# ztlpn/minilp

Hardware: AMD Instinct MI355X
Metric: simplex pivots/sec (higher is better)
Workload: dtype f64; 1 GPU; config 4: random LP 100000 vars x 100000 constraints, 100 nnz/row (0.1% fill), Max c'x, Ax<=b, x>=0; primal simplex with PSE+DSE from the slack basis; timed pivots 5..1983; parallelism=1 GPU, nucleus_size_at_end=1559, completed_steps=1978

## Files before the change

### minilp_amd/csrc/kernels.hip

```cpp
#include "kernels.h"
#include <hip/hip_ext.h>

#include <limits.h>
#include <math.h>

#include <cstdlib>
#include <string>

namespace mlp {

#define NONE_IDX INT_MAX
constexpr int BLK = 256;

struct Cand {
    double key;
    int idx;
};
__device__ __forceinline__ Cand cand_none() { return Cand{-INFINITY, NONE_IDX}; }
__device__ __forceinline__ bool cand_better(const Cand& a, const Cand& b) {
    return a.key > b.key || (a.key == b.key && a.idx < b.idx);
}
__device__ __forceinline__ Cand wave_best(Cand c) {
#pragma unroll
    for (int o = 32; o > 0; o >>= 1) {
// ... 711 lines not shown
            v.tau[r] = inv * inv;
        }
        int base = v.csr_ptr[i_r], end = v.csr_ptr[i_r + 1];
        int cnt = 0;
        for (int e0 = base; e0 < end; e0 += 128) {
            int sx[2] = {-1, -1}, cx[2], lx[2];
            double ax[2];
            bool vx[2];
#pragma unroll
            for (int h = 0; h < 2; ++h) {
                const int e = e0 + 64 * h + lane;
                vx[h] = e < end;
                cx[h] = vx[h] ? v.csr_col[e] : 0;
                ax[h] = vx[h] ? v.csr_val[e] : 0.0;
            }
#pragma unroll
            for (int h = 0; h < 2; ++h) lx[h] = v.var_loc[cx[h]];
#pragma unroll
            for (int h = 0; h < 2; ++h) {
                const int ks = v.kslot_of_pos[lx[h] >= 0 ? lx[h] : 0];
                if (vx[h] && lx[h] >= 0) sx[h] = ks;
            }
#pragma unroll
            for (int h = 0; h < 2; ++h) {
                if (h == 1 && e0 + 64 >= end) break;
                const int s = sx[h];
                bool isk = vx[h] && s >= 0;
                unsigned long long mask = __ballot(isk);
                const double coef = -ax[h] * inv;
                if (isk) {
                    int off = cnt + __popcll(mask & ((1ull << lane) - 1ull));
                    v.blist_s[off] = s;
                    v.blist_a[off] = coef;
                    if (l_n && off < RK_LDS) {
                        l_s[off] = s;
                        l_a[off] = coef;
                    }
                }
                cnt += __popcll(mask);
                if (nlow > 0) lr_dot_listed(mask, s, coef, Urow, lane < nlow, lr_acc);
            }
        }
        if (lane == 0) {
            it->blist_n = cnt;
            if (l_n) *l_n = cnt;
        }
    }
    if (nlow > 0) {
        if (sr >= 0 && lane < nlow) lr_acc = Urow[sr];
        if (lane < nlow) c->lr_e[lane] = lr_acc;
    }
    if (plan_after && lane == 0) plan_update(v, c, phase);
}

__device__ __forceinline__ Cand price_primal_one(double dd, double gm, uint8_t f, int j, int use_pse) {
    if (((f & NB_AT_MIN) && dd > -EPS) || ((f & NB_AT_MAX) && dd < EPS)) return cand_none();
    return Cand{use_pse ? dd * dd / gm : fabs(dd), j};
}
__device__ __forceinline__ Cand price_dual_one(double val, double mn, double mx, double bt, int r, int use_dse) {
    double infeas;
    if (val < mn - EPS) infeas = mn - val;
    else if (val > mx + EPS) infeas = val - mx;
    else return cand_none();
    return Cand{use_dse ? infeas * infeas / bt : infeas, r};
}
__device__ __forceinline__ void open_iteration(Ctl* c, int phase, Cand best) {
    IterState* it = &c->it;
    it->klist_n = 0;
    it->blist_n = 0;
    c->up.kase = -1;
    if (best.idx == NONE_IDX) {
        it->status = phase == 0 ? ITER_OPTIMAL : ITER_FEASIBLE;
        it->q = -1;
        it->r = -1;
        c->halt = 1;
        push_rec(c, phase);
    } else {
        it->status = ITER_PIVOT;
        if (phase == 0) {
            it->q = best.idx;
            it->r = -1;
        } else {
            it->r = best.idx;
            it->q = -1;
        }
    }
}
__device__ __forceinline__ void close_and_open(const DevView& v, Ctl* c, int phase, Cand best, double pay, bool close_current) {
    __shared__ double s_key, s_pay;
    __shared__ int s_idx, s_go;
    if (threadIdx.x == 0) {
        if (close_current) push_rec(c, phase);
        if (close_current && v.str_on) {
            c->hyper_epoch += 1;
            c->str_n = 0;
            c->aq_n = 0;
        }
        s_go = 1;
        if (close_current && c->forced) {
            c->halt = 1;
            s_go = 0;
        }
        s_key = best.key;
        s_idx = best.idx;
        s_pay = pay;
    }
    __syncthreads();
    if (!s_go || threadIdx.x >= 64) return;
    Cand b{s_key, s_idx};
    bool ok = true;
    if (phase == 0) ok = exchange_best_wave(v, c, phase, b, s_pay, threadIdx.x);
    else if (threadIdx.x == 0) ok = adopt_rank0_candidate(v, c, b);
    if (threadIdx.x == 0 && ok) open_iteration(c, phase, b);
}
__global__ void __launch_bounds__(BLK) k_price_primal(DevView v, int use_pse) {
    Ctl* c = v.ctl;
    if (c->halt) return;
    Cand best = cand_none();
    double pay = 0.0;
    for (int j = v.nb_lo + blockIdx.x * BLK + threadIdx.x; j < v.nb_hi; j += gridDim.x * BLK) {
        double dj = v.d[j];
        Cand t = price_primal_one(dj, use_pse ? v.gamma[j] : 1.0, v.nbflags[j], j, use_pse);
        if (cand_better(t, best)) {
            best = t;
            pay = dj;
        }
    }
    if (!grid_best_p(best, pay, v)) return;
    close_and_open(v, c, 0, best, pay, false);
}
__global__ void __launch_bounds__(BLK) k_price_dual(DevView v, int use_dse) {
    Ctl* c = v.ctl;
    if (c->halt || c->forced) return;
    Cand best = cand_none();
    for (int r = blockIdx.x * BLK + threadIdx.x; r < v.m; r += gridDim.x * BLK) {
        Cand t = price_dual_one(v.xB[r], v.loB[r], v.hiB[r], use_dse ? v.beta[r] : 1.0, r, use_dse);
        if (cand_better(t, best)) best = t;
    }
    if (!grid_best(best, v)) return;
    if (threadIdx.x == 0 && adopt_rank0_candidate(v, c, best)) open_iteration(c, 1, best);
}

__global__ void __launch_bounds__(64) k_ftran_prep(DevView v, int derive_primal) {
    Ctl* c = v.ctl;
    if (c->halt || c->it.status != ITER_PIVOT) {
        if (threadIdx.x == 0) c->side_go = 0;
        return;
    }
    if (threadIdx.x == 0) c->side_go = 1;
    KMARK0(c, 0);
    ftran_prep_wave(v, c, threadIdx.x, derive_primal);
}
template <int G>
__device__ __forceinline__ void push_F(const DevView& v, int p, double x, double* out_pos, int gl, Ctl* list_ctl = nullptr) {
    int var = v.basic_vars[p];
    int end = v.csc_ptr[var + 1];
    for (int e = v.csc_ptr[var] + gl; e < end; e += G) {
        const RowInfo ri = v.rowinfo[v.csc_row[e]];
        if (ri.kslot < 0) {
            unsafeAtomicAdd(&out_pos[ri.pos], -v.csc_val[e] * x / ri.diag);
            if (list_ctl) aq_list_add(v, list_ctl, ri.pos);
        }
    }
}
template <int G>
__device__ __forceinline__ void mark_F(const DevView& v, int p, int gl) {
    const int var = v.basic_vars[p];
    const int end = v.csc_ptr[var + 1];
    for (int e = v.csc_ptr[var] + gl; e < end; e += G) {
        const RowInfo ri = v.rowinfo[v.csc_row[e]];
        if (ri.kslot < 0) v.fmark[ri.pos] = 1;
    }
}
template <int G>
__global__ void __launch_bounds__(BLK) k_ftran_gather(DevView v) {
    Ctl* c = v.ctl;
    if (c->halt || c->it.status != ITER_PIVOT) return;
    KMARK0(c, 18);
    int slot = (blockIdx.x * BLK + threadIdx.x) / G;
    int gl = threadIdx.x & (G - 1);
    if (slot >= c->k) return;
    int n = c->it.klist_n;
    double acc = 0.0;
    const double* wrow = v.W + (size_t)slot * v.ld;
    if (G == 4) {
        for (int j0 = gl; j0 < n; j0 += 16) {
            double a[4], w[4];
            int si[4];
#pragma unroll
            for (int u = 0; u < 4; ++u) {
                const int j = j0 + 4 * u;
                a[u] = j < n ? v.klist_a[j] : 0.0;
                si[u] = j < n ? v.klist_s[j] : 0;
            }
#pragma unroll
            for (int u = 0; u < 4; ++u) w[u] = j0 + 4 * u < n ? wrow[si[u]] : 0.0;
#pragma unroll
            for (int u = 0; u < 4; ++u)
                if (j0 + 4 * u < n) acc += a[u] * w[u];
        }
        if (v.lrJ) {
            const int nlow = c->nlow;
            double e[LR_MAX / 4], x[LR_MAX / 4];
#pragma unroll
            for (int u = 0; u < LR_MAX / 4; ++u) {
                const int j = gl + 4 * u;
                e[u] = j < nlow ? c->lr_c[j] : 0.0;
                x[u] = j < nlow ? v.U[(size_t)j * v.ld + slot] : 0.0;
            }
#pragma unroll
            for (int u = 0; u < LR_MAX / 4; ++u)
                if (gl + 4 * u < nlow) acc += x[u] * e[u];
        }
    } else {
        for (int j = gl; j < n; j += G) acc += v.klist_a[j] * wrow[v.klist_s[j]];
        if (v.lrJ) {
            const int nlow = c->nlow;
            for (int j = gl; j < nlow; j += G) acc += v.U[(size_t)j * v.ld + slot] * c->lr_c[j];
        }
    }
    acc = group_sum<G>(acc);
    int p = v.pos_of_kslot[slot];
    if (gl == 0) {
        v.aK[slot] = acc;
        v.alpha_q[p] = acc;
        if (acc != 0.0 && aq_listing(v)) aq_list_add(v, c, p);
    }
    if (acc != 0.0 && !v.pb_on && !v.det_pull) push_F<G>(v, p, acc, v.alpha_q, gl, aq_listing(v) ? c : nullptr);
    else if (acc != 0.0 && v.det_pull && v.fmark) mark_F<G>(v, p, gl);
}

constexpr int PB_TILE = 512;
__global__ void __launch_bounds__(BLK) k_push_stage1(DevView v, int which) {
    Ctl* c = v.ctl;
    if (c->halt || c->it.status != ITER_PIVOT) return;
    KMARK0(c, 19);
    __shared__ double acc[PB_ROWS];
    __shared__ double s_x[PB_TILE];
    __shared__ int s_beg[PB_TILE], s_len[PB_TILE];
    int b = blockIdx.x, cc = blockIdx.y;
    if ((gridDim.y & 7) == 0) {
        const int L = (int)blockIdx.x + (int)gridDim.x * (int)blockIdx.y, idx = L >> 3;
        cc = (L & 7) + 8 * (idx / (int)gridDim.x);
        b = idx % (int)gridDim.x;
    }
    const int tid = threadIdx.x;
    const int row0 = b * PB_ROWS;
    const int nrows = min(PB_ROWS, v.m - row0);
    for (int t = tid; t < nrows; t += BLK) acc[t] = 0.0;
    const int k = c->k;
    const int per = (k + (int)gridDim.y - 1) / (int)gridDim.y;
    const int s_lo = cc * per, s_hi = min(k, s_lo + per);
    const double* xK = which ? v.tauK : v.aK;
    const int lane = tid & 7, grp = tid >> 3;
    const int stride = v.pb_rb + 1;
    for (int tile0 = s_lo; tile0 < s_hi; tile0 += PB_TILE) {
        const int nt = min(PB_TILE, s_hi - tile0);
        __syncthreads();
        for (int t = tid; t < nt; t += BLK) {
            const int slot = tile0 + t;
            const double x = xK[slot];
            const int var = v.basic_vars[v.pos_of_kslot[slot]];
            const int beg = v.colblk[(size_t)var * stride + b], end = v.colblk[(size_t)var * stride + b + 1];
            s_x[t] = x;
            s_beg[t] = beg;
            s_len[t] = (x != 0.0) ? end - beg : 0;
        }
        __syncthreads();
        for (int base = grp * 4; base < nt; base += (BLK / 8) * 4) {
            int r[4];
            double a[4];
#pragma unroll
            for (int j = 0; j < 4; ++j) {
                const int t = base + j;
                const int len = t < nt ? s_len[t] : 0;
                r[j] = -1;
                a[j] = 0.0;
                if (lane < len) {
                    const int e = s_beg[t] + lane;
                    r[j] = v.csc_row[e] - row0;
                    a[j] = v.csc_val[e] * s_x[t];
                }
            }
#pragma unroll
            for (int j = 0; j < 4; ++j)
                if (r[j] >= 0) unsafeAtomicAdd(&acc[r[j]], a[j]);
#pragma unroll 1
            for (int j = 0; j < 4; ++j) {
                const int t = base + j;
                const int len = t < nt ? s_len[t] : 0;
                for (int o = 8 + lane; o < len; o += 8) {
                    const int e = s_beg[t] + o;
                    unsafeAtomicAdd(&acc[v.csc_row[e] - row0], v.csc_val[e] * s_x[t]);
                }
            }
        }
    }
    __syncthreads();
    double* dst = v.push_part + (size_t)cc * v.m + row0;
    for (int t = tid; t < nrows; t += BLK) dst[t] = acc[t];
}
constexpr int PBD_TILE = 256;
constexpr int PBD_CHUNKS_DEFAULT = 16;
constexpr size_t PBD_LDS = sizeof(unsigned long long) * 2 * PB_ROWS + sizeof(double) * PBD_TILE + sizeof(int) * 2 * PBD_TILE;
__global__ void __launch_bounds__(BLK) k_push_stage1_det(DevView v, int which) {
    Ctl* c = v.ctl;
    if (c->halt || c->it.status != ITER_PIVOT) return;
    KMARK0(c, 19);
    extern __shared__ unsigned long long s_pbd[];
    unsigned long long* accH = s_pbd;
    unsigned long long* accL = s_pbd + PB_ROWS;
    double* s_x = reinterpret_cast<double*>(s_pbd + 2 * PB_ROWS);
    int* s_beg = reinterpret_cast<int*>(s_x + PBD_TILE);
    int* s_len = s_beg + PBD_TILE;
    __shared__ double s_bound;
    int b = blockIdx.x, cc = blockIdx.y;
// ... 790 lines not shown
            c->it.max_step = max_step;
            c->it.alpha_sq = sq + 1.0;
            st_agent(&c->ratio_max_step, max_step);
            __hip_atomic_store(v.ticket, 0u, __ATOMIC_RELAXED, __HIP_MEMORY_SCOPE_AGENT);
            asm volatile("s_waitcnt vmcnt(0)" ::: "memory");
            st_agent(&c->ratio_epoch, epoch0 + 1);
        }
    }
    __shared__ int s_gave_up;
    if (threadIdx.x == 0) {
        s_gave_up = 0;
        long spins = 0;
        while (ld_agent(&c->ratio_epoch) != epoch0 + 1) {
            __builtin_amdgcn_s_sleep(1);
            if (++spins > c->ratio_spin_limit) {
                s_gave_up = 1;
                break;
            }
        }
        s_max_step = ld_agent(&c->ratio_max_step);
    }
    __syncthreads();
    if (s_gave_up) {
        if (threadIdx.x == 0 && atomicExch(&c->halt, 1) == 0) {
            c->it.status = ITER_STALL;
            push_rec(c, 0);
        }
        return;
    }
    const double max_step = s_max_step;
#pragma unroll
    for (int u = 0; u < PT; ++u) {
        if (pos[u] < 0) continue;
        if (stp[u] / ca[u] <= max_step) {
            Cand t{ca[u], pos[u]};
            if (cand_better(t, best)) best = t;
        }
    }
    if (!grid_best(best, v, nrb)) return;
    } while (0);
    ratio_primal_finish(v, c, best, rk_inside);
    KMARK(c, 6);
}

__global__ void __launch_bounds__(BLK) k_post_ftran(DevView v, int use_pse) {
    Ctl* c = v.ctl;
    if (c->halt || c->it.status != ITER_PIVOT) return;
    double sq = 0.0;
    if (use_pse) {
        for (int p = blockIdx.x * BLK + threadIdx.x; p < v.m; p += gridDim.x * BLK) {
            double coeff = v.alpha_q[p];
            sq += coeff * coeff;
            if (!v.fac_on && v.kslot_of_pos[p] < 0) v.rv[v.srow_of_pos[p]].y = coeff / v.sdiag_of_pos[p];
        }
    }
    if (!grid_sum(sq, v)) return;
    if (threadIdx.x == 0) {
        c->it.alpha_sq = sq + 1.0;
        plan_update(v, c, 1);
    }
}

__global__ void __launch_bounds__(64) k_btran_prep(DevView v, int derive_dual, int plan_after) {
    Ctl* c = v.ctl;
    if (c->halt || c->it.status != ITER_PIVOT) return;
    btran_prep_wave(v, c, threadIdx.x, c->it.r, derive_dual, plan_after, 1);
}
__device__ __forceinline__ void btran_rk_body(const DevView& v, Ctl* c, int block, int n_gather, int after_fold) {
    const int k = c->k;
    const int n = c->it.blist_n;
    double sq = 0.0;
    if (v.lrJ) {
        const int nlow = (after_fold && c->fold) ? 0 : c->nlow;
        for (int g4 = block * BLK + (int)threadIdx.x; g4 < 4 * k; g4 += n_gather * BLK) {
            const int s = g4 >> 2, gl = g4 & 3;
            double acc = 0.0;
            for (int j0 = gl; j0 < n; j0 += 16) {
                double a[4], w[4];
                int si[4];
#pragma unroll
                for (int u = 0; u < 4; ++u) {
                    const int j = j0 + 4 * u;
                    a[u] = j < n ? v.blist_a[j] : 0.0;
                    si[u] = j < n ? v.blist_s[j] : 0;
                }
#pragma unroll
                for (int u = 0; u < 4; ++u) w[u] = j0 + 4 * u < n ? v.W[(size_t)si[u] * v.ld + s] : 0.0;
#pragma unroll
                for (int u = 0; u < 4; ++u)
                    if (j0 + 4 * u < n) acc += a[u] * w[u];
            }
            {
                double e[LR_MAX / 4], x[LR_MAX / 4];
#pragma unroll
                for (int u = 0; u < LR_MAX / 4; ++u) {
                    const int j = gl + 4 * u;
                    e[u] = j < nlow ? c->lr_e[j] : 0.0;
                    x[u] = j < nlow ? v.V[(size_t)j * v.ld + s] : 0.0;
                }
#pragma unroll
                for (int u = 0; u < LR_MAX / 4; ++u)
                    if (gl + 4 * u < nlow) acc += e[u] * x[u];
            }
            acc += __shfl_xor(acc, 1, 64);
            acc += __shfl_xor(acc, 2, 64);
            if (gl == 0) {
                v.rK[s] = acc;
                v.rv[v.row_of_kslot[s]].x = acc;
                sq += acc * acc;
            }
        }
    } else
    for (int s = block * BLK + (int)threadIdx.x; s < k; s += n_gather * BLK) {
        double acc = 0.0;
        for (int j = 0; j < n; ++j) acc += v.blist_a[j] * v.W[(size_t)v.blist_s[j] * v.ld + s];
        v.rK[s] = acc;
        v.rv[v.row_of_kslot[s]].x = acc;
        sq += acc * acc;
    }
    if (!grid_sum(sq, v, n_gather, block)) return;
    if (threadIdx.x == 0) {
        int r = c->it.r;
        if (v.kslot_of_pos[r] < 0) {
            double inv = 1.0 / v.sdiag_of_pos[r];
            sq += inv * inv;
        }
        c->it.rho_sq = sq;
    }
}
template <int G>
__global__ void __launch_bounds__(BLK) k_btran(DevView v, int n_gather, int after_fold = 0) {
    Ctl* c = v.ctl;
    if (c->halt || c->it.status != ITER_PIVOT) return;
    KMARK0(c, 7);
    const int k = c->k;
    if ((int)blockIdx.x < n_gather) {
        btran_rk_body(v, c, (int)blockIdx.x, n_gather, after_fold);
    } else {
        int slot = (((int)blockIdx.x - n_gather) * BLK + threadIdx.x) / G;
        int gl = threadIdx.x & (G - 1);
        if (slot >= k) return;
        int p = v.pos_of_kslot[slot];
        int var = v.basic_vars[p];
        int end = v.csc_ptr[var + 1];
        double acc = 0.0;
        for (int e = v.csc_ptr[var] + gl; e < end; e += G) acc += v.csc_val[e] * v.rv[v.csc_row[e]].y;
        acc = group_sum<G>(acc);
        if (gl == 0) v.tK[slot] = v.alpha_q[p] - acc;
    }
}


constexpr int HEAD_CAP = 1024;
__device__ void ftran_head_lds(const DevView& v, Ctl* c, int lane, int derive_primal, bool primary, int* ls, double* la, int* ln) {
    IterState* it = &c->it;
    const int q = it->q;
    const int var = v.nb_vars[q];
    if (primary && lane == 0) {
        it->entering_var = var;
        if (derive_primal) {
            double dq = v.d[q];
            it->sign = dq < 0.0;
            it->entering_cur = v.xN[q];
            it->entering_other = (dq < 0.0) ? v.var_hi[var] : v.var_lo[var];
            it->r = -1;
            it->leaving_var = -1;
        }
    }
    const bool atomic_land = !v.pb_on && !v.det_pull;
    const int base = v.csc_ptr[var], end = v.csc_ptr[var + 1];
    int cnt = 0;
    for (int e0 = base; e0 < end; e0 += 64) {
        const int e = e0 + lane;
        const bool valid = e < end;
        int s = -1;
        double a = 0.0;
        if (valid) {
            const int i = v.csc_row[e];
            a = v.csc_val[e];
            s = v.kslot_of_row[i];
            if (s < 0 && primary) {
                const int p = v.pos_of_srow[i];
                const double x = a / v.sdiag_of_pos[p];
                if (atomic_land) unsafeAtomicAdd(&v.alpha_q[p], x);
                else v.alpha_q[p] = x;
                if (aq_listing(v)) aq_list_add(v, c, p);
            }
        }
        const bool isk = valid && s >= 0;
        const unsigned long long mask = __ballot(isk);
        if (isk) {
            const int off = cnt + __popcll(mask & ((1ull << lane) - 1ull));
            if (off < HEAD_CAP) {
                ls[off] = s;
                la[off] = a;
            }
            if (primary) {
                v.klist_s[off] = s;
                v.klist_a[off] = a;
            }
        }
        cnt += __popcll(mask);
    }
    if (lane == 0) {
        *ln = cnt < HEAD_CAP ? cnt : HEAD_CAP;
        if (primary) it->klist_n = cnt;
    }
}
__global__ void __launch_bounds__(BLK) k_ftran_gather_lrh(DevView v, int fpk) {
    Ctl* c = v.ctl;
    if (c->halt || c->it.status != ITER_PIVOT) {
        if (blockIdx.x == 0 && threadIdx.x == 0) c->side_go = 0;
        return;
    }
    KMARK0(c, 0);
    __shared__ int s_ls[HEAD_CAP];
    __shared__ double s_la[HEAD_CAP];
    __shared__ double s_lrc[LR_MAX];
    __shared__ int s_n;
    const bool primary = blockIdx.x == 0;
    const int nlow = c->nlow;
    if (threadIdx.x < 64) {
        const int lane = threadIdx.x;
        IterState* it = &c->it;
        const int q = it->q;
        const int var = v.nb_vars[q];
        if (primary && lane == 0) {
            c->side_go = 1;
            it->entering_var = var;
            const double dq = v.d[q];
            it->sign = dq < 0.0;
            it->entering_cur = v.xN[q];
            it->entering_other = (dq < 0.0) ? v.var_hi[var] : v.var_lo[var];
            it->r = -1;
            it->leaving_var = -1;
            c->fold = nlow >= v.lrJ ? 1 : 0;
        }
        const int base = v.csc_ptr[var], end = v.csc_ptr[var + 1];
        int cnt = 0;
        const double* Vrow = v.V + (size_t)(lane < nlow ? lane : 0) * v.ld;
        double lr_acc = 0.0;
        for (int e0 = base; e0 < end; e0 += 128) {
            int sx[2] = {-1, -1};
            double ax[2] = {0.0, 0.0};
            int ix[2];
            bool vx[2];
#pragma unroll
            for (int h = 0; h < 2; ++h) {
                const int e = e0 + 64 * h + lane;
                vx[h] = e < end;
                ix[h] = vx[h] ? v.csc_row[e] : 0;
                ax[h] = vx[h] ? v.csc_val[e] : 0.0;
            }
            RowInfo rx[2];
#pragma unroll
            for (int h = 0; h < 2; ++h) rx[h] = v.rowinfo[ix[h]];
#pragma unroll
            for (int h = 0; h < 2; ++h) {
                if (vx[h]) {
                    sx[h] = rx[h].kslot;
                    if (sx[h] < 0 && primary) v.alpha_q[rx[h].pos] = ax[h] / rx[h].diag;
                }
            }
#pragma unroll
            for (int h = 0; h < 2; ++h) {
                if (h == 1 && e0 + 64 >= end) break;
                const int s = sx[h];
                const double a = ax[h];
                const bool isk = vx[h] && s >= 0;
                const unsigned long long mask = __ballot(isk);
                if (isk) {
                    const int off = cnt + __popcll(mask & ((1ull << lane) - 1ull));
                    if (off < HEAD_CAP) {
                        s_ls[off] = s;
                        s_la[off] = a;
                    }
                    if (primary) {
                        v.klist_s[off] = s;
                        v.klist_a[off] = a;
                    }
                }
                cnt += __popcll(mask);
                if (nlow > 0) lr_dot_listed(mask, s, a, Vrow, lane < nlow, lr_acc);
            }
        }
        if (lane == 0) {
            s_n = cnt < HEAD_CAP ? cnt : HEAD_CAP;
            if (primary) it->klist_n = cnt;
        }
        if (lane < LR_MAX) s_lrc[lane] = lane < nlow ? lr_acc : 0.0;
        if (primary && lane < nlow) c->lr_c[lane] = lr_acc;
    }
    __syncthreads();
    const int slot = (blockIdx.x * BLK + threadIdx.x) / 4;
    const int gl = threadIdx.x & 3;
    if (slot >= c->k) return;
    const int n = s_n;
    double acc = 0.0;
    const double* wrow = v.W + (size_t)slot * v.ld;
    const int p = v.pos_of_kslot[slot];
    const int fvar = fpk ? v.basic_vars[p] : 0;
    for (int j0 = gl; j0 < n; j0 += 16) {
        double a[4], w[4];
        int si[4];
#pragma unroll
        for (int u = 0; u < 4; ++u) {
            const int j = j0 + 4 * u;
            a[u] = j < n ? s_la[j] : 0.0;
            si[u] = j < n ? s_ls[j] : 0;
        }
#pragma unroll
        for (int u = 0; u < 4; ++u) w[u] = j0 + 4 * u < n ? wrow[si[u]] : 0.0;
#pragma unroll
        for (int u = 0; u < 4; ++u)
            if (j0 + 4 * u < n) acc += a[u] * w[u];
    }
    {
        double e[LR_MAX / 4], x[LR_MAX / 4];
#pragma unroll
        for (int u = 0; u < LR_MAX / 4; ++u) {
            const int j = gl + 4 * u;
            e[u] = j < nlow ? s_lrc[j] : 0.0;
            x[u] = j < nlow ? v.U[(size_t)j * v.ld + slot] : 0.0;
        }
#pragma unroll
        for (int u = 0; u < LR_MAX / 4; ++u)
            if (gl + 4 * u < nlow) acc += x[u] * e[u];
    }
    acc = group_sum<4>(acc);
    if (gl == 0) {
        v.aK[slot] = acc;
        v.alpha_q[p] = acc;
        if (fpk) v.fpk_x[fvar] = acc;
    }
}
template <int G>
__global__ void __launch_bounds__(BLK) k_ftran_fused(DevView v, int derive_primal) {
    Ctl* c = v.ctl;
    if (c->halt || c->it.status != ITER_PIVOT) return;
    KMARK0(c, 0);
    __shared__ int s_ls[HEAD_CAP];
    __shared__ double s_la[HEAD_CAP];
    __shared__ int s_n;
    if (threadIdx.x < 64) ftran_head_lds(v, c, threadIdx.x, derive_primal, blockIdx.x == 0, s_ls, s_la, &s_n);
    __syncthreads();
    const int slot = (blockIdx.x * BLK + threadIdx.x) / G;
    const int gl = threadIdx.x & (G - 1);
    if (slot >= c->k) return;
    const int n = s_n;
    double acc = 0.0;
    const double* wrow = v.W + (size_t)slot * v.ld;
    for (int j = gl; j < n; j += G) acc += s_la[j] * wrow[s_ls[j]];
    acc = group_sum<G>(acc);
    const int p = v.pos_of_kslot[slot];
    if (gl == 0) {
        v.aK[slot] = acc;
        v.alpha_q[p] = acc;
        if (acc != 0.0 && aq_listing(v)) aq_list_add(v, c, p);
    }
    if (acc != 0.0 && !v.pb_on && !v.det_pull) push_F<G>(v, p, acc, v.alpha_q, gl, aq_listing(v) ? c : nullptr);
    else if (acc != 0.0 && v.det_pull && v.fmark) mark_F<G>(v, p, gl);
}
__device__ void btran_head_lds(const DevView& v, Ctl* c, int lane, int derive_dual, bool primary, int* ls, double* la, int* ln) {
    IterState* it = &c->it;
    const int r = it->r;
    if (derive_dual && !c->forced && primary && lane == 0) {
        const double val = v.xB[r], mn = v.loB[r];
        it->leaving_new_val = (val < mn) ? mn : v.hiB[r];
        it->leaving_var = v.basic_vars[r];
        it->q = -1;
        it->entering_var = -1;
    }
    const int sr = v.kslot_of_pos[r];
    if (sr >= 0) {
        if (lane == 0) {
            ls[0] = sr;
            la[0] = 1.0;
            *ln = 1;
            if (primary) {
                v.blist_s[0] = sr;
                v.blist_a[0] = 1.0;
                it->blist_n = 1;
            }
        }
        return;
    }
    const int i_r = v.srow_of_pos[r];
    const double inv = 1.0 / v.sdiag_of_pos[r];
    if (primary && lane == 0) {
        v.rv[i_r].x = inv;
        v.tau[r] = inv * inv;
    }
    const int base = v.csr_ptr[i_r], end = v.csr_ptr[i_r + 1];
    int cnt = 0;
    for (int e0 = base; e0 < end; e0 += 64) {
        const int e = e0 + lane;
        const bool valid = e < end;
        int s = -1;
        double a = 0.0;
        if (valid) {
            const int loc = v.var_loc[v.csr_col[e]];
            a = v.csr_val[e];
            if (loc >= 0) s = v.kslot_of_pos[loc];
        }
        const bool isk = valid && s >= 0;
        const unsigned long long mask = __ballot(isk);
        if (isk) {
            const int off = cnt + __popcll(mask & ((1ull << lane) - 1ull));
            if (off < HEAD_CAP) {
                ls[off] = s;
                la[off] = -a * inv;
            }
            if (primary) {
                v.blist_s[off] = s;
                v.blist_a[off] = -a * inv;
            }
        }
        cnt += __popcll(mask);
    }
    if (lane == 0) {
        *ln = cnt < HEAD_CAP ? cnt : HEAD_CAP;
        if (primary) it->blist_n = cnt;
    }
}
template <int G>
__global__ void __launch_bounds__(BLK) k_btran_fused(DevView v, int n_gather, int derive_dual) {
    Ctl* c = v.ctl;
    if (c->halt || c->it.status != ITER_PIVOT) return;
    const int k = c->k;
    if ((int)blockIdx.x < n_gather) {
        __shared__ int s_ls[HEAD_CAP];
        __shared__ double s_la[HEAD_CAP];
        __shared__ int s_n;
        if (threadIdx.x < 64) btran_head_lds(v, c, threadIdx.x, derive_dual, blockIdx.x == 0, s_ls, s_la, &s_n);
        __syncthreads();
        const int n = s_n;
        double sq = 0.0;
        for (int s = blockIdx.x * BLK + threadIdx.x; s < k; s += n_gather * BLK) {
            double acc = 0.0;
            for (int j = 0; j < n; ++j) acc += s_la[j] * v.W[(size_t)s_ls[j] * v.ld + s];
            v.rK[s] = acc;
            v.rv[v.row_of_kslot[s]].x = acc;
            sq += acc * acc;
        }
        if (!grid_sum(sq, v, n_gather)) return;
        if (threadIdx.x == 0) {
            const int r = c->it.r;
            if (v.kslot_of_pos[r] < 0) {
                const double inv = 1.0 / v.sdiag_of_pos[r];
                sq += inv * inv;
            }
            c->it.rho_sq = sq;
        }
    } else {
        const int slot = (((int)blockIdx.x - n_gather) * BLK + threadIdx.x) / G;
        const int gl = threadIdx.x & (G - 1);
        if (slot >= k) return;
        const int p = v.pos_of_kslot[slot];
        const int var = v.basic_vars[p];
        const int end = v.csc_ptr[var + 1];
        double acc = 0.0;
        for (int e = v.csc_ptr[var] + gl; e < end; e += G) {
            const int i = v.csc_row[e];
            if (v.kslot_of_row[i] < 0) acc += v.csc_val[e] * v.rv[i].y;
        }
        acc = group_sum<G>(acc);
        if (gl == 0) v.tK[slot] = v.alpha_q[p] - acc;
    }
}

__device__ __forceinline__ void lowrank_append(const DevView& v, Ctl* c, const StructUpdate& u, int s) {
    const int kold = u.kold, ld = v.ld, last = kold - 1;
    const double inv_alpha = c->it.inv_alpha;
    const int jn = u.jn;
    if (u.kase == 4) {
        if (s == 0) c->nlow = jn;
        return;
    }
    double* Un = v.U + (size_t)jn * ld;
    double* Vn = v.V + (size_t)jn * ld;
    if (u.kase == 0 || u.kase == 2) {
        const int lim = (u.kase == 2) ? last : kold;
        if (s < lim) {
            int sr_src = (u.kase == 2 && s == u.sr) ? last : s;
            int sc_src = (u.kase == 2 && s == u.cq) ? last : s;
            const double un = -(v.aK[sr_src] - (sr_src == u.sr ? 1.0 : 0.0)) * inv_alpha;
            Un[s] = un;
            v.Ut[(size_t)s * LR_MAX + jn] = un;
            Vn[s] = v.rK[sc_src];
        }
        if (u.kase == 2 && s < jn) {
            double* Uj = v.U + (size_t)s * ld;
            double* Vj = v.V + (size_t)s * ld;
            if (u.sr != last) {
                const double x = Uj[last];
                Uj[u.sr] = x;
                v.Ut[(size_t)u.sr * LR_MAX + s] = x;
            }
            if (u.cq != last) Vj[u.cq] = Vj[last];
        }
    } else if (u.kase == 1) {
        if (s < kold) {
            const double un = -v.aK[s] * inv_alpha;
            Un[s] = un;
            v.Ut[(size_t)s * LR_MAX + jn] = un;
            Vn[s] = v.rK[s];
        } else if (s == kold) {
            Un[kold] = 0.0;
            v.Ut[(size_t)kold * LR_MAX + jn] = 0.0;
            Vn[kold] = 0.0;
        }
        if (s < jn) {
            v.U[(size_t)s * ld + kold] = 0.0;
            v.Ut[(size_t)kold * LR_MAX + s] = 0.0;
// ... 521 lines not shown
        const int j = v.nb_lo + (int)blockIdx.x * BLK + threadIdx.x + u * (int)gridDim.x * BLK;
        pos[u] = -1;
        ca[u] = 0.0;
        dj[u] = 0.0;
        if (j >= v.nb_hi) continue;
        const double coeff = v.alpha_r[j];
        const uint8_t f = v.nbflags[j];
        if (!dual_eligible(coeff, f, lsign)) continue;
        pos[u] = j;
        ca[u] = fabs(coeff);
        dj[u] = fabs(clamp_obj(v.d[j], f));
        const double cur = (dj[u] + EPS) / ca[u];
        if (cur < mn) mn = cur;
    }
    __shared__ double s_step;
    __shared__ int s_state;
    if (grid_min_sum(mn, dummy, v)) {
        if (threadIdx.x == 0) s_step = mn;
        __syncthreads();
        bool ok = true;
        double g = s_step;
        if (threadIdx.x < 64) ok = exchange_min_wave(v, c, g, threadIdx.x);
        if (threadIdx.x == 0) {
            if (ok) it->max_step = g;
            st_agent(&c->ratio_max_step, ok ? g : -1.0);
            __hip_atomic_store(v.ticket, 0u, __ATOMIC_RELAXED, __HIP_MEMORY_SCOPE_AGENT);
            asm volatile("s_waitcnt vmcnt(0)" ::: "memory");
            st_agent(&c->ratio_epoch, epoch0 + 1);
        }
    }
    if (threadIdx.x == 0) {
        int state = 0;
        long spins = 0;
        while (ld_agent(&c->ratio_epoch) != epoch0 + 1) {
            __builtin_amdgcn_s_sleep(1);
            if (++spins > c->ratio_spin_limit) {
                state = 1;
                break;
            }
        }
        const double stp = ld_agent(&c->ratio_max_step);
        if (state == 0 && stp < 0.0) state = 2;
        s_step = stp;
        s_state = state;
    }
    __syncthreads();
    if (s_state) {
        if (s_state == 1 && threadIdx.x == 0 && atomicExch(&c->halt, 1) == 0) {
            it->status = ITER_STALL;
            push_rec(c, 1);
        }
        return;
    }
    const double max_step = s_step;
    Cand best = cand_none();
#pragma unroll
    for (int u = 0; u < PT; ++u) {
        if (pos[u] < 0) continue;
        if (dj[u] / ca[u] <= max_step) {
            Cand t{ca[u], pos[u]};
            if (cand_better(t, best)) best = t;
        }
    }
    if (!grid_best(best, v)) return;
    ratio_dual_finish(v, c, best, ar);
}
template <int G>
__global__ void __launch_bounds__(BLK) k_btran_rhs(DevView v) {
    Ctl* c = v.ctl;
    if (c->halt || c->it.status != ITER_PIVOT) return;
    int slot = (blockIdx.x * BLK + threadIdx.x) / G;
    int gl = threadIdx.x & (G - 1);
    if (slot >= c->k) return;
    int p = v.pos_of_kslot[slot];
    int var = v.basic_vars[p];
    int end = v.csc_ptr[var + 1];
    double acc = 0.0;
    for (int e = v.csc_ptr[var] + gl; e < end; e += G) acc += v.csc_val[e] * v.rv[v.csc_row[e]].y;
    acc = group_sum<G>(acc);
    if (gl == 0) v.tK[slot] = v.alpha_q[p] - acc;
}

typedef double dbl2_t __attribute__((ext_vector_type(2)));
template <bool NT>
__device__ __forceinline__ double2 fw_load2(const double* p) {
    if (NT) {
        dbl2_t t = __builtin_nontemporal_load(reinterpret_cast<const dbl2_t*>(p));
        return make_double2(t.x, t.y);
    }
    return *reinterpret_cast<const double2*>(p);
}
template <bool NT>
__device__ __forceinline__ void fw_store2(double* p, double a, double b) {
    if (NT) {
        dbl2_t t = {a, b};
        __builtin_nontemporal_store(t, reinterpret_cast<dbl2_t*>(p));
    } else {
        *reinterpret_cast<double2*>(p) = make_double2(a, b);
    }
}
template <int TR, bool WITH_TAU, bool WITH_V, bool DO_UPDATE, bool NT = false, bool LR = false, int RL = 1, bool TILED = false>
__global__ void __launch_bounds__(BLK) k_fused_w(DevView v) {
    Ctl* c = v.ctl;
    if (c->halt || c->it.status != ITER_PIVOT) return;
    KMARK0(c, 8);
    if (LR && c->fold) return;
    const int k = c->k, ld = v.ld;
    const int n_tile_blocks = TILED ? (int)gridDim.x - (LR ? LR_MAX : 0) : 0;
    if (LR && (TILED ? (int)blockIdx.x >= n_tile_blocks : blockIdx.y == gridDim.y - 1)) {
        const int j = TILED ? (int)blockIdx.x - n_tile_blocks : (int)blockIdx.x;
        if (j >= c->nlow) return;
        const double* Vj = v.V + (size_t)j * ld;
        const double* Uj = v.U + (size_t)j * ld;
        double g = 0.0, h = 0.0;
        for (int s = threadIdx.x; s < k; s += BLK) {
            g += Vj[s] * v.rK[s];
            if (WITH_V) h += Uj[s] * v.tK[s];
        }
        g = block_sum(g);
        h = block_sum(h);
        if (threadIdx.x == 0) {
            c->lr_g[j] = g;
            c->lr_h[j] = h;
        }
        return;
    }
    __shared__ double s_tau[TR * RL][BLK / 64];
    const int tid = threadIdx.x;
    const int nchunks_k = (k + FW_TC - 1) / FW_TC;
    const int ntiles = TILED ? ((k + TR * RL - 1) / (TR * RL)) * nchunks_k : 1;
    for (int tile = TILED ? (int)blockIdx.x : 0; tile < ntiles; tile += TILED ? n_tile_blocks : 1) {
    const int stripe = TILED ? tile / nchunks_k : (int)blockIdx.x;
    const int chunk = TILED ? tile % nchunks_k : (int)blockIdx.y;
    const int row0 = stripe * (TR * RL);
    const int col0 = chunk * FW_TC;
    if (row0 >= k || col0 >= k) return;
    int cidx[4];
    cidx[0] = col0 + 2 * tid;
    cidx[1] = cidx[0] + 1;
    cidx[2] = col0 + 512 + 2 * tid;
    cidx[3] = cidx[2] + 1;
    double rk[4];
#pragma unroll
    for (int j = 0; j < 4; ++j) rk[j] = (cidx[j] < k) ? v.rK[cidx[j]] : 0.0;
    const double inv_alpha = DO_UPDATE ? c->it.inv_alpha : 0.0;
    const int rslot = DO_UPDATE ? c->up.sr : -1;
    double vacc[4] = {0.0, 0.0, 0.0, 0.0};
    const bool pair0 = cidx[1] < k, pair1 = cidx[3] < k;
    const bool one0 = cidx[0] < k, one1 = cidx[2] < k;
    const int wv = tid >> 6, l = tid & 63;
#pragma unroll 1
    for (int sub = 0; sub < RL; ++sub) {
        double tacc[TR];
#pragma unroll
        for (int a = 0; a < TR; ++a) {
            int row = row0 + sub * TR + a;
            tacc[a] = 0.0;
            if (row >= k) continue;
            double* wp = v.W + (size_t)row * ld;
            double w[4] = {0.0, 0.0, 0.0, 0.0};
            if (pair0) {
                double2 t = fw_load2<NT>(wp + cidx[0]);
                w[0] = t.x;
                w[1] = t.y;
            } else if (one0) {
                w[0] = wp[cidx[0]];
            }
            if (pair1) {
                double2 t = fw_load2<NT>(wp + cidx[2]);
                w[2] = t.x;
                w[3] = t.y;
            } else if (one1) {
                w[2] = wp[cidx[2]];
            }
            if (WITH_TAU) tacc[a] = w[0] * rk[0] + w[1] * rk[1] + w[2] * rk[2] + w[3] * rk[3];
            if (WITH_V) {
                double t = v.tK[row];
#pragma unroll
                for (int j = 0; j < 4; ++j) vacc[j] += w[j] * t;
            }
            if (DO_UPDATE) {
                double u = (v.aK[row] - (row == rslot ? 1.0 : 0.0)) * inv_alpha;
#pragma unroll
                for (int j = 0; j < 4; ++j) w[j] -= u * rk[j];
                if (pair0) fw_store2<NT>(wp + cidx[0], w[0], w[1]);
                else if (one0) wp[cidx[0]] = w[0];
                if (pair1) fw_store2<NT>(wp + cidx[2], w[2], w[3]);
                else if (one1) wp[cidx[2]] = w[2];
            }
        }
        if (WITH_TAU) {
#pragma unroll
            for (int a = 0; a < TR; ++a) {
                double sacc = wave_sum(tacc[a]);
                if (l == 0) s_tau[sub * TR + a][wv] = sacc;
            }
        }
    }
    if (WITH_V) {
        double* pv = v.part_v + (size_t)stripe * ld;
#pragma unroll
        for (int j = 0; j < 4; ++j)
            if (cidx[j] < k) pv[cidx[j]] = vacc[j];
    }
    if (WITH_TAU) {
        __syncthreads();
        for (int t = tid; t < TR * RL; t += BLK) {
            int row = row0 + t;
            if (row < k) {
                double sacc = s_tau[t][0];
                for (int i = 1; i < BLK / 64; ++i) sacc += s_tau[t][i];
                v.part_tau[(size_t)chunk * ld + row] = sacc;
            }
        }
    }
    if (TILED) __syncthreads();
    }
}
template <int TR, bool WITH_V, bool NT, int RL = 1>
__global__ void __launch_bounds__(BLK) k_fused_lr(DevView v, int fold_only) {
    Ctl* c = v.ctl;
    if (!fold_only && (c->halt || c->it.status != ITER_PIVOT)) return;
    const int k = c->k, ld = v.ld;
    const int nlow = c->nlow;
    const bool fold = fold_only || c->fold;
    if (!fold) return;
    const int tid = threadIdx.x;
    const int row0 = blockIdx.x * (TR * RL);
    const int col0 = blockIdx.y * FW_TC;
    if (row0 >= k || col0 >= k) return;
    __shared__ double s_tau[TR * RL][BLK / 64];
    __shared__ double s_u[LR_MAX][TR];
    int cidx[4];
    cidx[0] = col0 + 2 * tid;
    cidx[1] = cidx[0] + 1;
    cidx[2] = col0 + 512 + 2 * tid;
    cidx[3] = cidx[2] + 1;
    const bool pair0 = cidx[1] < k, pair1 = cidx[3] < k;
    const bool one0 = cidx[0] < k, one1 = cidx[2] < k;
    double rk[4];
#pragma unroll
    for (int q = 0; q < 4; ++q) rk[q] = (!fold_only && cidx[q] < k) ? v.rK[cidx[q]] : 0.0;
    double vacc[4] = {0.0, 0.0, 0.0, 0.0};
    const int wv = tid >> 6, l = tid & 63;
#pragma unroll 1
    for (int sub = 0; sub < RL; ++sub) {
        const int rbase = row0 + sub * TR;
        if (rbase >= k) break;
        double w[TR][4];
#pragma unroll
        for (int a = 0; a < TR; ++a) {
            int row = rbase + a;
            w[a][0] = w[a][1] = w[a][2] = w[a][3] = 0.0;
            if (row >= k) continue;
            const double* wp = v.W + (size_t)row * ld;
            if (pair0) {
                double2 t = fw_load2<NT>(wp + cidx[0]);
                w[a][0] = t.x;
                w[a][1] = t.y;
            } else if (one0) {
                w[a][0] = wp[cidx[0]];
            }
            if (pair1) {
                double2 t = fw_load2<NT>(wp + cidx[2]);
                w[a][2] = t.x;
                w[a][3] = t.y;
            } else if (one1) {
                w[a][2] = wp[cidx[2]];
            }
        }
        if (nlow > 0) {
            __syncthreads();
            for (int i = tid; i < nlow * TR; i += BLK) {
                int j = i / TR, a = i % TR;
                int row = rbase + a;
                s_u[j][a] = row < k ? v.U[(size_t)j * ld + row] : 0.0;
            }
            __syncthreads();
            for (int j = 0; j < nlow; ++j) {
                const double* Vj = v.V + (size_t)j * ld;
                double vj[4];
#pragma unroll
                for (int q = 0; q < 4; ++q) vj[q] = (cidx[q] < k) ? Vj[cidx[q]] : 0.0;
#pragma unroll
                for (int a = 0; a < TR; ++a) {
                    double u = s_u[j][a];
#pragma unroll
                    for (int q = 0; q < 4; ++q) w[a][q] += u * vj[q];
                }
            }
#pragma unroll
            for (int a = 0; a < TR; ++a) {
                int row = rbase + a;
                if (row >= k) continue;
                double* wp = v.W + (size_t)row * ld;
                if (pair0) fw_store2<NT>(wp + cidx[0], w[a][0], w[a][1]);
                else if (one0) wp[cidx[0]] = w[a][0];
                if (pair1) fw_store2<NT>(wp + cidx[2], w[a][2], w[a][3]);
                else if (one1) wp[cidx[2]] = w[a][2];
            }
        }
        if (fold_only) continue;
#pragma unroll
        for (int a = 0; a < TR; ++a) {
            int row = rbase + a;
            double tacc = w[a][0] * rk[0] + w[a][1] * rk[1] + w[a][2] * rk[2] + w[a][3] * rk[3];
            if (WITH_V && row < k) {
                double t = v.tK[row];
#pragma unroll
                for (int q = 0; q < 4; ++q) vacc[q] += w[a][q] * t;
            }
            double sacc = wave_sum(tacc);
            if (l == 0) s_tau[sub * TR + a][wv] = sacc;
        }
    }
    if (fold_only) return;
    if (WITH_V) {
        double* pv = v.part_v + (size_t)blockIdx.x * ld;
#pragma unroll
        for (int q = 0; q < 4; ++q)
            if (cidx[q] < k) pv[cidx[q]] = vacc[q];
    }
    __syncthreads();
    for (int t = tid; t < TR * RL; t += BLK) {
        int row = row0 + t;
        if (row < k) {
            double sacc = s_tau[t][0];
            for (int i = 1; i < BLK / 64; ++i) sacc += s_tau[t][i];
            v.part_tau[(size_t)blockIdx.y * ld + row] = sacc;
        }
    }
}

constexpr int SW_MAX_BLOCKS = 8192;
static int fold_max_blocks() {
    return SW_MAX_BLOCKS;
}
__device__ __forceinline__ int sw_strip_rows(const DevView& v, int k, int ch, int rs, int rb_fixed) {
    if (!v.sw_nbal || rb_fixed != 128) return rb_fixed;
    const int nch = (k + ch - 1) / ch;
    const int mult = v.wshard ? v.world : 1;
// ... 1834 lines not shown
```

Measured before the change: 11190 pivots/s.

## Prefetch FTRAN push entries before head sync and batch W-update row loads

In the fused FTRAN kernel, each thread now loads its slot's column pointers, first CSC entries and row info before the head phase and the barrier. This hides that load latency behind the head work, and the push loop uses the preloaded entries first. In the W update kernel, each group of 8 rows now issues all its W, tK and aK loads up front, clamped to valid rows, before the compute and store phase. This raises memory-level parallelism at the cost of more registers and some redundant loads on edge tiles.

```diff
diff --git a/minilp_amd/csrc/kernels.hip b/minilp_amd/csrc/kernels.hip
--- a/minilp_amd/csrc/kernels.hip
+++ b/minilp_amd/csrc/kernels.hip
@@ -887,16 +887,20 @@
     ftran_prep_wave(v, c, threadIdx.x, derive_primal);
 }
 template <int G>
-__device__ __forceinline__ void push_F(const DevView& v, int p, double x, double* out_pos, int gl, Ctl* list_ctl = nullptr) {
-    int var = v.basic_vars[p];
-    int end = v.csc_ptr[var + 1];
-    for (int e = v.csc_ptr[var] + gl; e < end; e += G) {
+__device__ __forceinline__ void push_F_entries(const DevView& v, int e, int end, double x, double* out_pos, Ctl* list_ctl) {
+    for (; e < end; e += G) {
         const RowInfo ri = v.rowinfo[v.csc_row[e]];
         if (ri.kslot < 0) {
             unsafeAtomicAdd(&out_pos[ri.pos], -v.csc_val[e] * x / ri.diag);
             if (list_ctl) aq_list_add(v, list_ctl, ri.pos);
         }
     }
+}
+template <int G>
+__device__ __forceinline__ void push_F(const DevView& v, int p, double x, double* out_pos, int gl, Ctl* list_ctl = nullptr) {
+    int var = v.basic_vars[p];
+    int end = v.csc_ptr[var + 1];
+    push_F_entries<G>(v, v.csc_ptr[var] + gl, end, x, out_pos, list_ctl);
 }
 template <int G>
 __device__ __forceinline__ void mark_F(const DevView& v, int p, int gl) {
@@ -1993,10 +1997,9 @@
 
 
 constexpr int HEAD_CAP = 1024;
-__device__ void ftran_head_lds(const DevView& v, Ctl* c, int lane, int derive_primal, bool primary, int* ls, double* la, int* ln) {
+__device__ void ftran_head_lds(const DevView& v, Ctl* c, int lane, int derive_primal, bool primary, int q, int var, int base, int end, int* ls,
+                               double* la, int* ln) {
     IterState* it = &c->it;
-    const int q = it->q;
-    const int var = v.nb_vars[q];
     if (primary && lane == 0) {
         it->entering_var = var;
         if (derive_primal) {
@@ -2009,7 +2012,6 @@
         }
     }
     const bool atomic_land = !v.pb_on && !v.det_pull;
-    const int base = v.csc_ptr[var], end = v.csc_ptr[var + 1];
     int cnt = 0;
     for (int e0 = base; e0 < end; e0 += 64) {
         const int e = e0 + lane;
@@ -2177,30 +2179,68 @@
 }
 template <int G>
 __global__ void __launch_bounds__(BLK) k_ftran_fused(DevView v, int derive_primal) {
+    constexpr int FP_E = 2;
     Ctl* c = v.ctl;
-    if (c->halt || c->it.status != ITER_PIVOT) return;
+    const int halt = c->halt, status = c->it.status, k = c->k, q = c->it.q;
+    if (halt || status != ITER_PIVOT) return;
     KMARK0(c, 0);
     __shared__ int s_ls[HEAD_CAP];
     __shared__ double s_la[HEAD_CAP];
     __shared__ int s_n;
-    if (threadIdx.x < 64) ftran_head_lds(v, c, threadIdx.x, derive_primal, blockIdx.x == 0, s_ls, s_la, &s_n);
-    __syncthreads();
     const int slot = (blockIdx.x * BLK + threadIdx.x) / G;
     const int gl = threadIdx.x & (G - 1);
-    if (slot >= c->k) return;
+    const bool head = threadIdx.x < 64, live = slot < k;
+    const bool push = live && !v.pb_on && !v.det_pull;
+    const int p = live ? v.pos_of_kslot[slot] : 0;
+    const int qvar = head ? v.nb_vars[q] : 0;
+    const int fvar = push ? v.basic_vars[p] : 0;
+    int qbase = 0, qend = 0, e0 = 0, fend = 0;
+    if (head) {
+        qbase = v.csc_ptr[qvar];
+        qend = v.csc_ptr[qvar + 1];
+    }
+    if (push) {
+        e0 = v.csc_ptr[fvar] + gl;
+        fend = v.csc_ptr[fvar + 1];
+    }
+    int frow[FP_E];
+    double fval[FP_E];
+    RowInfo fri[FP_E];
+#pragma unroll
+    for (int u = 0; u < FP_E; ++u) {
+        const bool in = e0 + u * G < fend;
+        frow[u] = in ? v.csc_row[e0 + u * G] : -1;
+        fval[u] = in ? v.csc_val[e0 + u * G] : 0.0;
+    }
+#pragma unroll
+    for (int u = 0; u < FP_E; ++u) {
+        fri[u] = RowInfo{0.0, -1, 0};
+        if (frow[u] >= 0) fri[u] = v.rowinfo[frow[u]];
+    }
+    if (head) ftran_head_lds(v, c, threadIdx.x, derive_primal, blockIdx.x == 0, q, qvar, qbase, qend, s_ls, s_la, &s_n);
+    __syncthreads();
+    if (!live) return;
     const int n = s_n;
     double acc = 0.0;
     const double* wrow = v.W + (size_t)slot * v.ld;
     for (int j = gl; j < n; j += G) acc += s_la[j] * wrow[s_ls[j]];
     acc = group_sum<G>(acc);
-    const int p = v.pos_of_kslot[slot];
     if (gl == 0) {
         v.aK[slot] = acc;
         v.alpha_q[p] = acc;
         if (acc != 0.0 && aq_listing(v)) aq_list_add(v, c, p);
     }
-    if (acc != 0.0 && !v.pb_on && !v.det_pull) push_F<G>(v, p, acc, v.alpha_q, gl, aq_listing(v) ? c : nullptr);
-    else if (acc != 0.0 && v.det_pull && v.fmark) mark_F<G>(v, p, gl);
+    if (acc != 0.0 && push) {
+        Ctl* list_ctl = aq_listing(v) ? c : nullptr;
+#pragma unroll
+        for (int u = 0; u < FP_E; ++u) {
+            if (frow[u] >= 0 && fri[u].kslot < 0) {
+                unsafeAtomicAdd(&v.alpha_q[fri[u].pos], -fval[u] * acc / fri[u].diag);
+                if (list_ctl) aq_list_add(v, list_ctl, fri[u].pos);
+            }
+        }
+        push_F_entries<G>(v, e0 + FP_E * G, fend, acc, v.alpha_q, list_ctl);
+    } else if (acc != 0.0 && v.det_pull && v.fmark) mark_F<G>(v, p, gl);
 }
 __device__ void btran_head_lds(const DevView& v, Ctl* c, int lane, int derive_dual, bool primary, int* ls, double* la, int* ln) {
     IterState* it = &c->it;
@@ -3028,41 +3068,72 @@
 #pragma unroll 1
     for (int sub = 0; sub < RL; ++sub) {
         double tacc[TR];
-#pragma unroll
-        for (int a = 0; a < TR; ++a) {
-            int row = row0 + sub * TR + a;
-            tacc[a] = 0.0;
-            if (row >= k) continue;
-            double* wp = v.W + (size_t)row * ld;
-            double w[4] = {0.0, 0.0, 0.0, 0.0};
-            if (pair0) {
-                double2 t = fw_load2<NT>(wp + cidx[0]);
-                w[0] = t.x;
-                w[1] = t.y;
-            } else if (one0) {
-                w[0] = wp[cidx[0]];
-            }
-            if (pair1) {
-                double2 t = fw_load2<NT>(wp + cidx[2]);
-                w[2] = t.x;
-                w[3] = t.y;
-            } else if (one1) {
-                w[2] = wp[cidx[2]];
-            }
-            if (WITH_TAU) tacc[a] = w[0] * rk[0] + w[1] * rk[1] + w[2] * rk[2] + w[3] * rk[3];
-            if (WITH_V) {
-                double t = v.tK[row];
-#pragma unroll
-                for (int j = 0; j < 4; ++j) vacc[j] += w[j] * t;
-            }
-            if (DO_UPDATE) {
-                double u = (v.aK[row] - (row == rslot ? 1.0 : 0.0)) * inv_alpha;
-#pragma unroll
-                for (int j = 0; j < 4; ++j) w[j] -= u * rk[j];
-                if (pair0) fw_store2<NT>(wp + cidx[0], w[0], w[1]);
-                else if (one0) wp[cidx[0]] = w[0];
-                if (pair1) fw_store2<NT>(wp + cidx[2], w[2], w[3]);
-                else if (one1) wp[cidx[2]] = w[2];
+        if constexpr (DO_UPDATE) {
+            constexpr int GR = 8;
+            const int c0 = one0 ? cidx[0] : col0, c2 = one1 ? cidx[2] : col0;
+#pragma unroll
+            for (int g0 = 0; g0 < TR; g0 += GR) {
+                double2 wa[GR], wb[GR];
+                double tk[GR], ak[GR];
+#pragma unroll
+                for (int a = 0; a < GR; ++a) {
+                    const int row = row0 + sub * TR + g0 + a;
+                    const int rc = row < k ? row : k - 1;
+                    const double* wp = v.W + (size_t)rc * ld;
+                    wa[a] = fw_load2<NT>(wp + c0);
+                    wb[a] = fw_load2<NT>(wp + c2);
+                    tk[a] = WITH_V ? v.tK[rc] : 0.0;
+                    ak[a] = v.aK[rc];
+                }
+#pragma unroll
+                for (int a = 0; a < GR; ++a) {
+                    const int row = row0 + sub * TR + g0 + a;
+                    tacc[g0 + a] = 0.0;
+                    if (row >= k) continue;
+                    double* wp = v.W + (size_t)row * ld;
+                    double w[4] = {one0 ? wa[a].x : 0.0, pair0 ? wa[a].y : 0.0, one1 ? wb[a].x : 0.0, pair1 ? wb[a].y : 0.0};
+                    if (WITH_TAU) tacc[g0 + a] = w[0] * rk[0] + w[1] * rk[1] + w[2] * rk[2] + w[3] * rk[3];
+                    if (WITH_V) {
+#pragma unroll
+                        for (int j = 0; j < 4; ++j) vacc[j] += w[j] * tk[a];
+                    }
+                    double u = (ak[a] - (row == rslot ? 1.0 : 0.0)) * inv_alpha;
+#pragma unroll
+                    for (int j = 0; j < 4; ++j) w[j] -= u * rk[j];
+                    if (pair0) fw_store2<NT>(wp + cidx[0], w[0], w[1]);
+                    else if (one0) wp[cidx[0]] = w[0];
+                    if (pair1) fw_store2<NT>(wp + cidx[2], w[2], w[3]);
+                    else if (one1) wp[cidx[2]] = w[2];
+                }
+            }
+        } else {
+#pragma unroll
+            for (int a = 0; a < TR; ++a) {
+                int row = row0 + sub * TR + a;
+                tacc[a] = 0.0;
+                if (row >= k) continue;
+                double* wp = v.W + (size_t)row * ld;
+                double w[4] = {0.0, 0.0, 0.0, 0.0};
+                if (pair0) {
+                    double2 t = fw_load2<NT>(wp + cidx[0]);
+                    w[0] = t.x;
+                    w[1] = t.y;
+                } else if (one0) {
+                    w[0] = wp[cidx[0]];
+                }
+                if (pair1) {
+                    double2 t = fw_load2<NT>(wp + cidx[2]);
+                    w[2] = t.x;
+                    w[3] = t.y;
+                } else if (one1) {
+                    w[2] = wp[cidx[2]];
+                }
+                if (WITH_TAU) tacc[a] = w[0] * rk[0] + w[1] * rk[1] + w[2] * rk[2] + w[3] * rk[3];
+                if (WITH_V) {
+                    double t = v.tK[row];
+#pragma unroll
+                    for (int j = 0; j < 4; ++j) vacc[j] += w[j] * t;
+                }
             }
         }
         if (WITH_TAU) {
```

Result: faster. 11590 pivots/s, median of 6 (+3.6%).
